# PoTaTo-Mika/fish-speech

Measured on AMD Instinct MI355X. Metric: audio-sec/wall-sec (RTF) + p50 first-sample latency, S2-Pro 4B @1/2/4/8 GPU, higher is better.
Workload: dtype bf16; 1 GPU; BASELINE config 2 per GPU: one utterance = 64-token prompt + 216 Dual-AR frames (top_k 30, top_p 0.8, temp 0.8) + codec decode [1,10,216] -> 442368 samples; global_batch=1, frames=216, prompt_len=64, first_chunk_frames=1, vocoder_chunks=first_chunk_frames, then growing 4x, vocoder=serial, parallelism=dp1

## Files before the change

fish-speech_amd/csrc/fm_kernels.h:

```cpp
#pragma once
#include <algorithm>
#include "fm_common.h"
#include "fm_tune_table.h"

enum { EPI_STORE = 0, EPI_RESID = 1, EPI_SWIGLU = 2, EPI_F32 = 3 };

template <typename T> void launch_swiglu_i8(hipStream_t s, const T* t, int ldt, T* act, int lda, int inter, int R);
template <typename T> void launch_pack(hipStream_t s, const T* src, int N, int K, T* dst);
template <typename T> void launch_quant_rows(hipStream_t s, T* w, int N, int K, int8_t* q, T* scale);
template <typename T> void launch_i8_to(hipStream_t s, const int8_t* q, int64_t n, T* dst);
void launch_pack_q8(hipStream_t s, const int8_t* src, int N, int K, int8_t* dst);
void launch_pack_q8s(hipStream_t s, const int8_t* src, int N, int K, int8_t* dst);
void launch_quant4(hipStream_t s, bf16_t* w, int N, int K, int gs, uint8_t* q, uint32_t* sz);
void launch_pack_q4(hipStream_t s, const uint8_t* q, int N, int K, uint8_t* dst);
void launch_pack_q4_rows(hipStream_t s, const uint8_t* q, int N, int K, uint32_t* dst);
void launch_pack_sz4(hipStream_t s, const uint32_t* sz, int N, int K, int gs, uint32_t* dst);
void launch_pack_q4s(hipStream_t s, const uint8_t* q, int N, int K, uint32_t* dst);

template <typename T> struct LinearArgs {
    const T* W;
    const T* W2;
    const T* bias;
    const T* X;
    int ldx, R, N, K;
// ... 212 lines not shown
    const bf16_t* nw;
    float eps;
    const bf16_t* res;
    int ldr;
    const int32_t* residx;
    int res_col, res_rows;
    bf16_t* res_out;
    bf16_t* Y;
    float* Yf;
    int N, K;
    const bf16_t* pf_kc;
    const bf16_t* pf_vc;
    const int32_t* pf_slot;
    const int32_t* pf_pos;
    size_t pf_slot_stride, pf_layer_off;
    int pf_S, pf_nkv, pf_hd;
    unsigned long long* dbg;
    int xr;
    const bf16_t* X1;
    const bf16_t* res1;
    bf16_t* res_out1;
    bf16_t* Y1;
    int skip0;
};
int rowgemv_u(int K, int qm);
void launch_rowgemv(hipStream_t s, const RowGemvArgs& a, int kind);
bool rowgemv_pair_ok(int kind, int K, bool gathered);
struct FattnWoArgs {
    FastFusedArgs<bf16_t> at;
    RowGemvArgs wo;
    uint32_t* xt;
    int gen;
    int* err;
    int delay;
    int cheap;
    int prio;
    int ilp;
    unsigned long long* dbg;
    const bf16_t* qtab;
    const int32_t* qidx;
    int qcol, qrows;
    int kv0;
    int pair;
};
bool fattn_wo_ok(int nh, int nkv, int hd, int cpos, int N, int K, int qm);
void launch_fattn_wo(hipStream_t s, const FattnWoArgs& a);
constexpr int GEMV_CHAIN_MAX = 4;
constexpr int GEMV_CHAIN_LINE = 32;
constexpr int GEMV_CHAIN_SLOTS = 17;
constexpr int GEMV_CHAIN_WORDS = GEMV_CHAIN_MAX * GEMV_CHAIN_SLOTS * GEMV_CHAIN_LINE;
enum { GEMV_CHAIN_WO_W2 = 0, GEMV_CHAIN_W13 = 1, GEMV_CHAIN_QKV = 2, GEMV_CHAIN_HEAD = 3 };
template <typename T> struct GemvChainArgs {
    GemvArgs<T> st[GEMV_CHAIN_MAX];
    int kind[GEMV_CHAIN_MAX];
    int off[GEMV_CHAIN_MAX + 1];
    int n;
    unsigned* cnt;
    int* err;
    int sleep;
};
template <typename T> void launch_gemv_chain(hipStream_t s, const GemvChainArgs<T>& c);

template <typename T> struct BstreamArgs {
    const T* W;
    const T* bias;
    const T* X;
    int ldx, R, N, K;
    T* Y;
// ... 115 lines not shown
```

fish-speech_amd/csrc/fm_llm_frame.cpp:

```cpp
#include <math.h>

#include <algorithm>
#include <array>

#include "fm_codec.h"
#include "fm_llm_model.h"

template <typename T> struct Run {
    typedef T type_t;
    fm_llm* m;
    hipStream_t s;
    int64_t E;
    bool rows_distinct_slots = false, bs_frame = false, x_ss = false;
    struct BsPending {
        bool on = false;
        const float* slab = nullptr;
        int kparts = 0, d = 0, R = 0;
        void* res = nullptr;
        void* out = nullptr;
        const void* sc = nullptr;
    } pend;
    std::vector<std::array<int, 2>> segs;
    void set_pending(const float* slab, int kparts, int d, int R, void* res, void* out, const void* sc) {
        pend = BsPending{true, slab, kparts, d, R, res, out, sc};
// ... 654 lines not shown
        int ldx_in;
        const int32_t* xidx;
        int xcol;
        void *xb, *hb;
        bool is_fast;
        int cpos, layer;
        KsbPlan kp;
        void* xo;
        int pair = 0;
        const void* x_in1 = nullptr;
    };
    static const void* row1(const Small& c, const void* p, int w) {
        return (const char*)p + (c.pair == 2 ? (size_t)w * sizeof(T) : 0);
    }
    static void* row1(const Small& c, void* p, int w) { return (char*)p + (c.pair == 2 ? (size_t)w * sizeof(T) : 0); }
    struct SmallPath {
        bool rf;
        bool fw;
        bool att_wo;
        bool row_here;
        bool tab;
        bool kv0;
        bool kv_only;
    };
    SmallPath small_path(const Small& c, bool kv_only) const {
        const StackDims& d = c.d;
        SmallPath p{};
        p.kv_only = kv_only;
        p.rf = row_fin(c.n);
        const int fq = m->quant == FM_QUANT_INT8 ? 1 : (m->quant == FM_QUANT_INT4 ? 2 : 0);
        p.fw = c.is_fast && !kv_only && p.rf && fm_tuning().fattn_wo && m->fxt && m->fdm.n_layer * m->C >= 2 &&
               m->fdm.n_layer * m->C <= 40 && fattn_wo_ok(d.nh, d.nkv, d.hd, c.cpos, d.dim, d.nq(), fq);
        p.att_wo = c.is_fast && !kv_only && fm_tuning().attn_wo && !m->quant && c.n == 1 && c.cpos < 16 && d.hd % 16 == 0 &&
                   d.hd <= 128 && d.nh % d.nkv == 0 && (d.nq() / c.kp.wo) % d.hd == 0 && d.nqkv() % 8 == 0;
        p.row_here = row_qkv(c.n) && (!c.first || (row_bits() & 16));
        const bool bits56 = sizeof(T) == 2 && !m->quant && c.is_fast && c.n == 1;
        p.tab = bits56 && c.first && c.xidx && p.fw && qkv0_live();
        p.kv0 = bits56 && c.cpos == 0 && (row_bits() & 64) && p.row_here && !p.att_wo && d.hd <= 256 &&
                (d.nqkv() - d.nq()) % fm_tuning().row_qkv_rp == 0;
        return p;
    }
    FastFusedArgs<T> small_fast_args(const Small& c, const SmallPath& p) const {
        const StackDims& d = c.d;
        FastFusedArgs<T> fa{(const T*)m->qkv, d.nqkv(), m->frame_slot, d.nh, d.nkv, d.hd, d.qk_norm,
                            m->c.norm_eps, (const T*)c.L.qn, (const T*)c.L.kn, m->frope, (T*)m->fkc,
                            (T*)m->fvc, m->fslot_stride, (size_t)c.layer * m->flayer_stride, m->C, c.cpos,
                            1.0f / sqrtf((float)d.hd), (T*)m->att};
        fa.dbg = fm_tuning().dbg;
        fa.noq = p.kv0;
        return fa;
    }
    void small_qkv(const Small& c, const SmallPath& p) {
        if (p.tab && !c.pair) return;
        const StackDims& d = c.d;
        GemvArgs<T> a = qkv_args(d, c.L, c.n);
        if (!c.is_fast && c.n == 1 && fm_tuning().kv_prefetch)
            kv_prefetch(a, (const T*)m->kc, (const T*)m->vc, m->frame_slot, m->frame_pos, m->slot_stride,
                        (size_t)c.layer * m->layer_stride, m->S, d.nkv, d.hd);
        else if (c.is_fast && c.n == 1 && fm_tuning().fkv_prefetch && m->fiota && c.cpos < 16)
            kv_prefetch(a, (const T*)m->fkc, (const T*)m->fvc, m->frame_slot, m->fiota + c.cpos, m->fslot_stride,
                        (size_t)c.layer * m->flayer_stride, m->C, d.nkv, d.hd);
        if (c.first) {
            qkv_first(d, c.L, a, c.n, c.x_in, c.ldx_in, c.pair ? nullptr : c.xidx, c.pair ? 0 : c.xcol, m->qkv,
                      p.kv0 || c.pair);
        } else if (p.row_here) {
            qkv_row(d, c.L, a, false, c.xb, 0, nullptr, 0, m->qkv, p.kv0, c.pair != 0);
        } else {
            a.X = (const T*)c.xb;
            a.ldx = d.dim;
            a.ss_in = m->ssX;
            a.ss_gran = p.rf ? 1 : 0;
            gemv(a, PRO_PRENORM, EPI_STORE, 1, "linear");
        }
    }
    void small_attn(const Small& c, const SmallPath& p) {
        const StackDims& d = c.d;
// ... 59 lines not shown
            if (!p.fw) {
                rowgemv(r, ROWGEMV_FIN);
                return;
            }
            const FastFusedArgs<T> fa = small_fast_args(c, p);
            A.at = *reinterpret_cast<const FastFusedArgs<bf16_t>*>(&fa);
            A.at.dbg = nullptr;
            A.at.row_pos = m->frame_pos;
            A.xt = m->fxt;
            A.gen = 1 + c.layer + m->fdm.n_layer * c.cpos;
            A.err = m->chain_err;
            A.delay = fm_tuning().fw_delay;
            A.cheap = fm_tuning().fw_cheap;
            A.prio = fm_tuning().fw_prio;
            A.ilp = fm_tuning().fattn_ilp;
            if (p.tab) {
                A.qtab = (const bf16_t*)m->qkv0;
                A.qidx = c.xidx;
                A.qcol = c.xcol;
                A.qrows = m->cb;
            }
            A.kv0 = p.kv0;
            A.pair = c.pair;
            hipStream_t st = s;
            auto go = [st, A] { launch_fattn_wo(st, A); };
            launch("attn", rowgemv_wbytes(r), 2.0 * r.N * r.K, go, "attn_wo");
            return;
        }
        GemvArgs<T> a = ga();
        a.W = (const T*)L.wo;
        a.bias = (const T*)L.bo;
        a.X = (const T*)m->att;
        a.ldx = d.nq();
        a.R = c.n;
        a.N = d.dim;
        a.K = d.nq();
        a.Yf = m->slabA;
        a.ldy = d.dim;
        if (c.first) {
            a.res = (const T*)c.x_in;
            a.ldr = c.ldx_in;
            a.residx = c.xidx;
            a.xidx_ld = m->C1;
            a.xidx_col = c.xcol;
            a.xidx_rows = c.xidx ? m->cb : 0;
        } else {
            a.res = (const T*)c.xb;
            a.ldr = d.dim;
        }
// ... 562 lines not shown
```

fish-speech_amd/csrc/fm_llm_model.h:

```cpp
#pragma once
#include <hip/hip_runtime.h>

#include "fm_kernels.h"
#include "fm_runtime.h"

static constexpr int PREFILL_CHUNK = 1024;
static constexpr int ATTN_PIECE = 256;
static constexpr int ATTN_SPLIT = 64;
static constexpr int GEMV_MAX_ROWS = 8;
static constexpr int KSB_MAX = 8;
static constexpr int BS_KPARTS = 8;

inline int pick_ksb(int N, int K, int R, size_t esz) {
    const int nb = (N + 15) / 16;
    const FmTuning& tu = fm_tuning();
    int ksb = 1;
    while (ksb < KSB_MAX && nb * ksb < tu.ksb_blocks && K % (32 * ksb * 2) == 0) ksb *= 2;
    if (tu.ksb_balance) {
        double best = 1e9;
        int bk = ksb;
        for (int k = 1; k <= KSB_MAX && K % (32 * k) == 0; k *= 2) {
            const int b = nb * k;
            if (b < 256) continue;
            const double rounds = (double)((b + 255) / 256), waste = rounds * 256.0 / b;
// ... 68 lines not shown
    bool use_graph = true;
    std::map<int, hipGraphExec_t> graphs;
    Profiler prof;
    std::vector<void*> allocs;
    int quant = FM_QUANT_NONE;
    int q4_gs = 0;
    int* fin_cnt = nullptr;
    float* fin_ss = nullptr;
    struct QInfo {
        const unsigned char* q8 = nullptr;
        const void* scale = nullptr;
        const uint32_t* sz = nullptr;
        const unsigned char* q8s = nullptr;
        const uint32_t* q4s = nullptr;
    };
    std::map<const void*, QInfo> qmap;
    std::map<const void*, void*> rowmajor;
    std::map<const void*, const void*> rowsz;
    std::map<const void*, const void*> rowscale;
    bool row_ok = false;
    bool row_qkv_ok = false;
    bool row_w13_ok = false;
    uint32_t* fxt = nullptr;
    void* fout_rm = nullptr;
    int32_t* fiota = nullptr;
    void* qkv0 = nullptr;
    int32_t* qkv0_iota = nullptr;
    unsigned qkv0_epoch = 0;
    bool qkv0_built = false;
    struct Prefix {
        void* buf = nullptr;
        int npos = 0;
        size_t bytes = 0;
    };
    std::map<int, Prefix> prefixes;
    int next_prefix_id = 1;
    int* pfx_slots = nullptr;
    const QInfo* qinfo(const void* W) const {
        auto it = qmap.find(W);
        return it == qmap.end() ? nullptr : &it->second;
    }

    ~fm_llm() {
        if (device >= 0) (void)hipSetDevice(device);
        for (auto& g : graphs) (void)hipGraphExecDestroy(g.second);
        for (auto& kv : w) {
// ... 37 lines not shown
```

fish-speech_amd/csrc/fm_llm_weights.cpp:

```cpp
#include "fm_llm_model.h"

void add_t(fm_llm* m, const std::string& n, int64_t rows, int64_t cols) {
    DTensor t;
    t.rows = rows;
    t.cols = cols;
    t.numel = rows * cols;
    m->w[n] = t;
}
static void add_stack(fm_llm* m, const std::string& pre, const StackDims& s) {
    for (int i = 0; i < s.n_layer; ++i) {
        std::string p = pre + std::to_string(i) + ".";
        add_t(m, p + "attention.wqkv.weight", s.nqkv(), s.dim);
        if (s.qkv_bias) add_t(m, p + "attention.wqkv.bias", 1, s.nqkv());
        add_t(m, p + "attention.wo.weight", s.dim, s.nq());
        if (s.o_bias) add_t(m, p + "attention.wo.bias", 1, s.dim);
        if (s.qk_norm) {
            add_t(m, p + "attention.q_norm.weight", 1, s.hd);
            add_t(m, p + "attention.k_norm.weight", 1, s.hd);
        }
        add_t(m, p + "feed_forward.w1.weight", s.inter, s.dim);
        add_t(m, p + "feed_forward.w3.weight", s.inter, s.dim);
        add_t(m, p + "feed_forward.w2.weight", s.dim, s.inter);
        add_t(m, p + "ffn_norm.weight", 1, s.dim);
        add_t(m, p + "attention_norm.weight", 1, s.dim);
// ... 337 lines not shown
            L.w2 = W(m, p + "feed_forward.w2.weight");
            L.an = W(m, p + "attention_norm.weight");
            L.fn = W(m, p + "ffn_norm.weight");
            auto rm = [&](const void* pk) -> void* {
                auto it = m->rowmajor.find(pk);
                return it == m->rowmajor.end() ? nullptr : it->second;
            };
            L.wo_rm = rm(L.wo);
            L.w2_rm = rm(L.w2);
            L.wqkv_rm = rm(L.wqkv);
            L.w13_rm = rm(L.w13);
        }
    };
    stack("layers.", m->sd, m->slow);
    stack("fast_layers.", m->fdm, m->fast);
    {
        int32_t io[16];
        for (int c = 0; c < 16; ++c) io[c] = c - 1;
        m->fiota = (int32_t*)m->dalloc(sizeof(io), false);
        HIPCHK(hipMemcpy(m->fiota, io, sizeof(io), hipMemcpyHostToDevice));
    }
    if (m->prec == FM_PREC_BF16)
        m->fxt = (uint32_t*)m->dalloc(2 * (size_t)m->fdm.nh * m->fdm.hd * sizeof(uint32_t));
    m->row_ok = m->row_qkv_ok = m->row_w13_ok = true;
    for (auto* st : {&m->slow, &m->fast})
        for (const LayerW& L : *st) {
            m->row_ok = m->row_ok && L.wo_rm && L.w2_rm;
            m->row_qkv_ok = m->row_qkv_ok && L.wqkv_rm;
            m->row_w13_ok = m->row_w13_ok && L.w13_rm;
        }
    if (m->quant) {
        for (auto* st : {&m->slow, &m->fast})
            for (LayerW& L : *st) L.bqkv = L.bo = nullptr;
    }
    m->emb = W(m, "embeddings.weight");
    m->cbemb = W(m, "codebook_embeddings.weight");
    m->norm = W(m, "norm.weight");
    m->fproj_w = Wopt(m, "fast_project_in.weight");
    m->fproj_b = m->quant ? nullptr : Wopt(m, "fast_project_in.bias");
    m->femb = W(m, "fast_embeddings.weight");
    m->fnorm = W(m, "fast_norm.weight");
    m->fout = W(m, "fast_output.weight");
    {
        auto it = m->rowmajor.find(m->fout);
        m->fout_rm = it == m->rowmajor.end() ? nullptr : it->second;
    }
// ... 138 lines not shown
```

fish-speech_amd/csrc/fm_rowgemv.hip:

```cpp
#include "fm_common.h"
#include "fm_kernels.h"
#include "fm_runtime.h"
#include <type_traits>

typedef __attribute__((ext_vector_type(2))) uint32_t u32x2_t;
typedef __attribute__((ext_vector_type(4))) __bf16 bf16x4_t;

__device__ __forceinline__ float dot4(u32x2_t w, u32x2_t x, float acc) {
    const bf16x4_t wb = __builtin_bit_cast(bf16x4_t, w), xb = __builtin_bit_cast(bf16x4_t, x);
    acc = __builtin_amdgcn_fdot2_f32_bf16(__builtin_shufflevector(wb, wb, 0, 1), __builtin_shufflevector(xb, xb, 0, 1),
                                          acc, false);
    acc = __builtin_amdgcn_fdot2_f32_bf16(__builtin_shufflevector(wb, wb, 2, 3), __builtin_shufflevector(xb, xb, 2, 3),
                                          acc, false);
    return acc;
}
__device__ __forceinline__ float lo16(uint32_t w) { return __uint_as_float(w << 16); }
__device__ __forceinline__ float hi16(uint32_t w) { return __uint_as_float(w & 0xffff0000u); }
__device__ __forceinline__ float dot8r(u32x4_t w, u32x4_t x, float acc) {
    const bf16x8_t wb = __builtin_bit_cast(bf16x8_t, w), xb = __builtin_bit_cast(bf16x8_t, x);
    acc = __builtin_amdgcn_fdot2_f32_bf16(__builtin_shufflevector(wb, wb, 0, 1), __builtin_shufflevector(xb, xb, 0, 1),
                                          acc, false);
    acc = __builtin_amdgcn_fdot2_f32_bf16(__builtin_shufflevector(wb, wb, 2, 3), __builtin_shufflevector(xb, xb, 2, 3),
                                          acc, false);
    acc = __builtin_amdgcn_fdot2_f32_bf16(__builtin_shufflevector(wb, wb, 4, 5), __builtin_shufflevector(xb, xb, 4, 5),
                                          acc, false);
    acc = __builtin_amdgcn_fdot2_f32_bf16(__builtin_shufflevector(wb, wb, 6, 7), __builtin_shufflevector(xb, xb, 6, 7),
                                          acc, false);
    return acc;
}
__device__ __forceinline__ void ld_pair_bf(const bf16_t* p, float& x0, float& x1) {
    const uint32_t w = *reinterpret_cast<const uint32_t*>(p);
    x0 = lo16(w);
    x1 = hi16(w);
}

template <int QM> struct RowT {
    static constexpr int EPL = QM ? 8 : 4;
    static constexpr int CE = 64 * EPL;
    using XV = typename std::conditional<QM != 0, u32x4_t, u32x2_t>::type;
    static constexpr int WPL = QM == 2 ? 1 : 2;
};

template <int U, int RP, bool PRENORM, int EPI, bool G, int QM, bool TX, int XR = 1>
__device__ __forceinline__ void rowgemv_body(const RowGemvArgs& a, const int blk, const uint32_t* xt, const uint32_t gen,
                                             int* err) {
    static_assert(!TX || (!PRENORM && EPI == 1), "tagged x: the residual form only");
    static_assert(XR == 1 || (XR == 2 && QM == 0 && EPI <= 1 && (!G || EPI == 1)), "two x rows: bf16 STORE / FIN");
    constexpr bool FIN = EPI == 1;
    using R = RowT<QM>;
    using XV = typename R::XV;
    constexpr int EPL = R::EPL, NW = EPL / 2;
    constexpr int SB = XR * 4 * RP;
    constexpr bool LATE = XR == 2 && !TX && !PRENORM && U >= 10;
    __shared__ float red[XR * (4 * RP + 8)];
    const int lane = threadIdx.x & 63, wave = threadIdx.x >> 6;
    const int n0 = blk * RP;
    const int nch = a.K / R::CE;
    const int wa = (wave * nch) >> 2, nmy = (((wave + 1) * nch) >> 2) - wa;
    const int last = nmy > 0 ? nmy - 1 : 0;
    const unsigned long long ts0 = a.dbg ? __builtin_amdgcn_s_memrealtime() : 0;
    const int er = n0 + (int)(threadIdx.x % RP);
    const int ex = XR == 2 ? (int)((threadIdx.x / RP) & 1) : 0;
    int ri = 0, xi = 0;
    if constexpr (G && FIN) {
        const int32_t iv = a.residx[a.res_col];
        ri = iv < 0 ? 0 : (iv >= a.res_rows ? a.res_rows - 1 : iv);
    } else if constexpr (G) {
        const int32_t iv = a.xidx[a.xcol];
        xi = iv < 0 ? 0 : (iv >= a.xrows ? a.xrows - 1 : iv);
    }
    bf16_t rv = 0;
    if constexpr (FIN && XR == 2) rv = ex ? a.res1[(size_t)ri * a.ldr + er] : a.res[er];
    else if constexpr (FIN) rv = a.res[(size_t)ri * a.ldr + er];
    const bf16_t bv = *(a.bias ? a.bias + er : a.X);
    bf16_t sv = 0;
    if constexpr (QM == 1) sv = a.wscale[er];
    const XV* xp = reinterpret_cast<const XV*>(a.X + (size_t)xi * a.ldx) + (size_t)wa * 64 + lane;
    const XV* gp = reinterpret_cast<const XV*>(PRENORM ? a.nw : a.X) + (size_t)wa * 64 + lane;
    XV xv[XR][U], gv[PRENORM ? U : 1];
    if constexpr (!TX) {
#pragma unroll
        for (int u = 0; u < U; ++u) {
            const int j = (u < last ? u : last) * 64;
            xv[0][u] = xp[j];
            if constexpr (XR == 2 && !LATE) xv[1][u] = (reinterpret_cast<const XV*>(a.X1) + (size_t)wa * 64 + lane)[j];
            if constexpr (PRENORM) gv[u] = gp[j];
        }
    }
    constexpr int PF = 2;
    const bool pf_on = EPI == 0 && a.pf_kc != nullptr;
    int pf_s = 0, pf_p = 0;
    if constexpr (EPI == 0) {
        pf_s = *(pf_on ? a.pf_slot : reinterpret_cast<const int32_t*>(a.X));
        pf_p = *(pf_on ? a.pf_pos : reinterpret_cast<const int32_t*>(a.X));
    }
    asm volatile("" ::: "memory");
    constexpr int WU = QM == 2 ? 1 : U, WR = QM == 2 ? 1 : RP;
    constexpr int QU = QM == 2 ? U : 1, QR = QM == 2 ? RP : 1;
    u32x2_t wv[WU][WR];
    uint32_t w4[QU][QR], szv[QU][QR];
    if constexpr (QM == 2) {
        const size_t rw = (size_t)(a.K >> 3);
        const int ng = a.K / a.gs;
        const uint32_t* wp = a.Wq4 + (size_t)n0 * rw + (size_t)wa * 64 + lane;
#pragma unroll
        for (int u = 0; u < U; ++u) {
            const int jc = u < last ? u : last;
#pragma unroll
            for (int r = 0; r < RP; ++r) {
                w4[u][r] = __builtin_nontemporal_load(wp + r * rw + jc * 64);
                szv[u][r] = a.wsz[(size_t)(n0 + r) * ng + ((wa + jc) * 512 + lane * 8) / a.gs];
            }
        }
    } else {
        const unsigned char* wb = QM ? reinterpret_cast<const unsigned char*>(a.Wq) : reinterpret_cast<const unsigned char*>(a.W);
        const size_t rowb = (size_t)a.K * (QM ? 1 : 2);
        const u32x2_t* wp = reinterpret_cast<const u32x2_t*>(wb + (size_t)n0 * rowb) + (size_t)wa * 64 + lane;
        const size_t rs8 = rowb / 8;
#pragma unroll
        for (int u = 0; u < U; ++u) {
            const int j = (u < last ? u : last) * 64;
#pragma unroll
            for (int r = 0; r < RP; ++r) wv[u][r] = __builtin_nontemporal_load(wp + r * rs8 + j);
        }
    }
    asm volatile("" ::: "memory");
    unsigned long long tsw = 0, tsx = 0;
    unsigned polls = 0;
    if constexpr (TX) {
        if (a.dbg) tsw = __builtin_amdgcn_s_memrealtime();
        const __amdgpu_buffer_rsrc_t xr = __builtin_amdgcn_make_buffer_rsrc((void*)xt, (short)0, XR * a.K * 4, 0x00020000);
        u32x4_t xw[XR][U][EPL / 4];
        for (unsigned it = 0;; ++it) {
            polls = it + 1;
#pragma unroll
            for (int x = 0; x < XR; ++x)
#pragma unroll
                for (int u = 0; u < U; ++u) {
                    const int jc = u < last ? u : last;
#pragma unroll
                    for (int q = 0; q < EPL / 4; ++q)
                        xw[x][u][q] = __builtin_amdgcn_raw_buffer_load_b128(
                            xr, (x * a.K + (wa + jc) * R::CE + EPL * lane + 4 * q) * 4, 0, 16);
                }
            bool ok = true;
#pragma unroll
// ... 3 lines not shown
#pragma unroll
                    for (int q = 0; q < EPL / 4; ++q)
#pragma unroll
                        for (int e = 0; e < 4; ++e) ok = ok && ((xw[x][u][q][e] & 0xffffu) == gen);
            if (__all(ok)) break;
            if (it >= (1u << 14)) {
                if (lane == 0) __hip_atomic_store(err, 1, __ATOMIC_RELAXED, __HIP_MEMORY_SCOPE_AGENT);
                break;
            }
            __builtin_amdgcn_s_sleep(1);
        }
        if (a.dbg) tsx = __builtin_amdgcn_s_memrealtime();
#pragma unroll
        for (int x = 0; x < XR; ++x)
#pragma unroll
            for (int u = 0; u < U; ++u)
#pragma unroll
                for (int h = 0; h < NW; ++h) {
                    const uint32_t w0 = xw[x][u][(2 * h) >> 2][(2 * h) & 3], w1 = xw[x][u][(2 * h + 1) >> 2][(2 * h + 1) & 3];
                    xv[x][u][h] = (w0 >> 16) | (w1 & 0xffff0000u);
                }
    }
    float pfw[PF];
    if constexpr (EPI == 0) {
        const char* kcb = reinterpret_cast<const char*>(pf_on ? a.pf_kc : a.X);
        const long long dv = pf_on ? reinterpret_cast<const char*>(a.pf_vc) - kcb : 0;
        const int nkv = pf_on ? a.pf_nkv : 1;
        const int b = blockIdx.x, h = b % nkv, jb = b / nkv, nb = ((int)gridDim.x - 1 - h) / nkv + 1;
        const int spr = pf_on ? a.pf_hd * 2 / 64 : 1;
        const int np = pf_on ? pf_p + 1 : 0, total = 2 * np * spr;
        const long long base = pf_on ? (long long)pf_s * (long long)a.pf_slot_stride + (long long)a.pf_layer_off +
                                           (long long)h * a.pf_S * a.pf_hd
                                     : 0;
#pragma unroll
        for (int q = 0; q < PF; ++q) {
            const int i = (jb + nb * q) * 256 + (int)threadIdx.x;
            const bool ok = i < total;
            const int ii = ok ? i : 0, row = ii / spr, sec = ii - row * spr;
            const bool isv = row >= np;
            const long long off = (isv ? dv : 0) + 2 * (base + (long long)(isv ? row - np : row) * a.pf_hd) + sec * 64;
            pfw[q] = *reinterpret_cast<const float*>(kcb + (ok ? off : 0));
        }
    }
    if constexpr (PRENORM && XR == 1) {
        float sl = 0.f;
#pragma unroll
        for (int u = 0; u < U; ++u) {
            if (u < nmy) {
#pragma unroll
                for (int h = 0; h < NW; ++h) {
                    const float e0 = lo16(xv[0][u][h]), e1 = hi16(xv[0][u][h]);
                    sl += e0 * e0 + e1 * e1;
                }
            }
        }
        sl = wave_sum(sl);
        if (lane == 0) red[4 * RP + wave] = sl;
        lds_barrier();
        const float tot = ((red[4 * RP] + red[4 * RP + 1]) + red[4 * RP + 2]) + red[4 * RP + 3];
        const float rs = 1.0f / sqrtf(tot / (float)a.K + a.eps);
#pragma unroll
        for (int u = 0; u < U; ++u) {
            XV o;
#pragma unroll
            for (int h = 0; h < NW; ++h) {
                const float y0 = bfround(bfround(lo16(xv[0][u][h]) * rs) * lo16(gv[u][h]));
                const float y1 = bfround(bfround(hi16(xv[0][u][h]) * rs) * hi16(gv[u][h]));
                o[h] = (uint32_t)f2bf(y0) | ((uint32_t)f2bf(y1) << 16);
            }
            xv[0][u] = o;
        }
    }
    if constexpr (PRENORM && XR == 2) {
#pragma unroll
        for (int x = 0; x < XR; ++x) {
            float sl = 0.f;
#pragma unroll
            for (int u = 0; u < U; ++u) {
                if (u < nmy) {
#pragma unroll
                    for (int h = 0; h < NW; ++h) {
                        const float e0 = lo16(xv[x][u][h]), e1 = hi16(xv[x][u][h]);
                        sl += e0 * e0 + e1 * e1;
// ... 64 lines not shown
#pragma unroll
                    for (int e = 0; e < 4; ++e) t = fmaf((float)((c0 >> (8 * e)) & 0xffu), xf[e], t);
#pragma unroll
                    for (int e = 0; e < 4; ++e) t = fmaf((float)((c1 >> (8 * e)) & 0xffu), xf[4 + e], t);
                    acc[0][r] = t;
                }
            }
        }
    }
    if constexpr (LATE) {
#pragma unroll
        for (int r = 0; r < RP; ++r) asm volatile("" : "+v"(acc[0][r])::"memory");
        const XV* xp1 = reinterpret_cast<const XV*>(a.X1) + (size_t)wa * 64 + lane;
#pragma unroll
        for (int u = 0; u < U; ++u) xv[1][u] = xp1[(u < last ? u : last) * 64];
#pragma unroll
        for (int u = 0; u < U; ++u) {
            if (u < nmy) {
#pragma unroll
                for (int r = 0; r < RP; ++r) acc[1][r] = dot4(wv[u][r], xv[1][u], acc[1][r]);
            }
        }
    }
    if constexpr (EPI == 0) {
#pragma unroll
        for (int q = 0; q < PF; ++q) asm volatile("" ::"v"(pfw[q]));
    }
    const unsigned long long ts1 = a.dbg ? __builtin_amdgcn_s_memrealtime() : 0;
#pragma unroll
    for (int x = 0; x < XR; ++x)
#pragma unroll
        for (int r = 0; r < RP; ++r) {
            const float v = wave_sum(acc[x][r]);
            if (lane == 0) red[(4 * x + wave) * RP + r] = v;
        }
    if constexpr (QM == 1) {
        const float v = wave_sum(xs);
        if (lane == 0) red[4 * RP + 4 + wave] = v;
    }
    __syncthreads();
    if ((int)threadIdx.x < XR * RP) {
        const int t = XR == 2 ? (int)(threadIdx.x % RP) : (int)threadIdx.x;
        const float* rd = red + 4 * RP * ex;
        float v = ((rd[t] + rd[RP + t]) + rd[2 * RP + t]) + rd[3 * RP + t];
        if constexpr (QM == 1) {
            const float xt = ((red[4 * RP + 4] + red[4 * RP + 5]) + red[4 * RP + 6]) + red[4 * RP + 7];
            v = bfround(bfround(v - 128.f * xt) * bf2f(sv));
        }
        if (a.bias) v += bf2f(bv);
        if constexpr (FIN) {
            (ex ? a.res_out1 : a.res_out)[er] = f2bf(bfround(bf2f(rv) + bfround(v)));
        } else if constexpr (EPI == 3) {
            a.Yf[er] = bfround(v);
        } else if constexpr (EPI == 2) {
            const float up = __shfl_down(v, RP / 2, 64);
            if (t < RP / 2) {
                const float g = bfround(v);
                a.Y[blockIdx.x * (RP / 2) + t] = f2bf(bfround(g / (1.0f + expf(-g))) * bfround(up));
            }
        } else if constexpr (XR == 2) {
            if (ex || er >= a.skip0) (ex ? a.Y1 : a.Y)[er] = f2bf(v);
        } else {
            a.Y[er] = f2bf(v);
        }
    }
    if (a.dbg && threadIdx.x == 0) {
#pragma unroll
        for (int x = 0; x < XR; ++x) {
            if constexpr (TX) {
                const unsigned long long t[7] = {ts0, tsw, tsx, ts1, __builtin_amdgcn_s_memrealtime(), 0, 0};
                dbg_record(a.dbg, 0xFFF8u, polls, t);
            } else {
                const unsigned long long t[7] = {ts0, ts1, __builtin_amdgcn_s_memrealtime(), 0, 0, 0, 0};
                dbg_record(a.dbg, 0xFFFAu, (unsigned)blk, t);
            }
        }
    }
}

template <int U, int RP, bool PRENORM, int EPI, bool G, int QM>
__global__ __launch_bounds__(256) __attribute__((amdgpu_waves_per_eu(RP == 2 ? 5 : 3)))
void rowgemv_kernel(RowGemvArgs a) {
    rowgemv_body<U, RP, PRENORM, EPI, G, QM, false>(a, blockIdx.x, nullptr, 0u, nullptr);
}
// ... 483 lines not shown
        fw_attend<2>(kvs, kvs + 2 * FW_MAXHD, hd, half, 1, lane, at.scale, q0, q1, k0, k1, v0, v1, o0, o1);
        const int K = at.nh * hd;
        if (in) {
            if constexpr (XR == 2) {
                const float p0 = 0.f + va0, p1 = 0.f + va1;
                const uint64_t w = (uint64_t)(((uint32_t)f2bf(p0) << 16) | gen) | ((uint64_t)(((uint32_t)f2bf(p1) << 16) | gen) << 32);
                __hip_atomic_store(reinterpret_cast<uint64_t*>(A.xt + (size_t)h * hd + 2 * lane), w, __ATOMIC_RELAXED,
                                   __HIP_MEMORY_SCOPE_AGENT);
            }
            const uint64_t w = (uint64_t)(((uint32_t)f2bf(o0) << 16) | gen) | ((uint64_t)(((uint32_t)f2bf(o1) << 16) | gen) << 32);
            __hip_atomic_store(reinterpret_cast<uint64_t*>(A.xt + K + (size_t)h * hd + 2 * lane), w, __ATOMIC_RELAXED,
                               __HIP_MEMORY_SCOPE_AGENT);
        }
        if (A.dbg && lane == 0) {
            const unsigned long long t[7] = {ts0, ts1, __builtin_amdgcn_s_memrealtime(), 0, 0, 0, 0};
#pragma unroll
            for (int x = 0; x < XR; ++x) dbg_record(A.dbg, 0xFFF9, (unsigned)h, t);
        }
        return;
    }
    rowgemv_body<U, 2, false, 1, TAB, 0, true, XR>(A.wo, (int)blockIdx.x - at.nkv, XR == 2 ? A.xt : A.xt + A.wo.K, gen, A.err);
}

bool fattn_wo_ok(int nh, int nkv, int hd, int cpos, int N, int K, int qm) {
    const int U = rowgemv_u(K, qm);
    return nkv > 0 && nh % nkv == 0 && nh / nkv <= 4 && hd % 2 == 0 && hd <= FW_MAXHD && cpos >= 0 &&
           cpos < FW_MAXJ + 1 && K == nh * hd && N % 2 == 0 && U > 0 && U <= 8;
}

void launch_fattn_wo(hipStream_t s, const FattnWoArgs& A0) {
    FattnWoArgs A = A0;
    A.dbg = fm_tuning().dbg;
    A.wo.dbg = A.dbg;
    const FastFusedArgs<bf16_t>& at = A.at;
    const int qm = A.wo.Wq4 ? 2 : (A.wo.Wq ? 1 : 0);
    FMCHECK(fattn_wo_ok(at.nh, at.nkv, at.hd, at.cpos, A.wo.N, A.wo.K, qm) && A.xt && A.err && A.gen > 0 && A.gen <= 40 && at.row_pos &&
                A.wo.res && A.wo.res_out &&
                (qm == 2 ? (A.wo.wsz && A.wo.gs % 8 == 0 && !A.wo.bias) : (qm == 1 ? (A.wo.wscale && !A.wo.bias) : A.wo.W != nullptr)),
            "fused fast attention + wo: shapes, tag and buffers");
    const dim3 grid(at.nkv + A.wo.N / 2), block(256);
    const bool G = A.wo.residx != nullptr;
    FMCHECK(!A.qtab || (qm == 0 && G && !A.kv0 && A.qidx == A.wo.residx && A.qcol == A.wo.res_col && A.qrows > 0 &&
                        A.qrows == A.wo.res_rows),
            "fused fast attention + wo: the QKV table form is bf16, gathered by the residual's index");
    FMCHECK(!A.kv0 || (qm == 0 && !G && at.cpos == 0), "fused fast attention + wo: the K / V-only form is bf16 at codebook 0");
    if (A.pair) {
        FMCHECK(qm == 0 && !A.kv0 && at.cpos == 1 && at.S >= 2 && rowgemv_pair_ok(-1, A.wo.K, false) && (A.qtab != nullptr) == G && (A.pair == 2 || (A.wo.res1 && A.wo.res_out1)),
                "fused fast attention + wo, pair form: bf16, positions 0 and 1, both rows' residuals set");
        const bool two = A.pair != 2;
        FMCHECK(two || !A.qtab, "fused fast attention + wo, pair form: the first layer is not the last");
        switch (rowgemv_u(A.wo.K, 0)) {
#define FW(u)                                                                                                            \
    case u:                                                                                                              \
        (A.qtab ? fattn_wo_pair_kernel<u, true, 2>                                                                       \
                : (two ? fattn_wo_pair_kernel<u, false, 2> : fattn_wo_pair_kernel<u, false, 1>))<<<grid, block, 0, s>>>(A); \
        break;
            FW(2) FW(3) FW(4)
            default: FW(5)
#undef FW
        }
        return;
    }
// ... 25 lines not shown
```

fish-speech_amd/csrc/fm_tune_table.h:

```cpp
#ifndef FM_TUNE_RULES
#define FM_TUNE_RULES
enum { FM_RULE_BOOL, FM_RULE_ANY, FM_RULE_SET, FM_RULE_RANGE, FM_RULE_MULT16 };
template <typename... V> constexpr int fm_knob_set(V... v) { return (0 | ... | (1 << v)); }
#define FM_BOOL FM_RULE_BOOL, 0, 0
#define FM_ANY FM_RULE_ANY, 0, 0
#define FM_SET(...) FM_RULE_SET, fm_knob_set(__VA_ARGS__), 0
#define FM_RANGE(lo, hi) FM_RULE_RANGE, lo, hi
#define FM_MIN(lo) FM_RULE_RANGE, lo, 0x7fffffff
#define FM_MULT16 FM_RULE_MULT16, 0, 0
#define FM_ZERO_OR_MULT16 FM_RULE_MULT16, 1, 0
#endif

#ifdef FM_KNOB
FM_KNOB(gemv_nt, 1, FM_BOOL)
FM_KNOB(gemv_u, 8, FM_SET(2, 4, 8))
FM_KNOB(gemv_wpb, 4, FM_SET(4, 8))
FM_KNOB(sampler_kth, 1, FM_BOOL)
FM_KNOB(sampler_fast, 1, FM_BOOL)
FM_KNOB(attn_cap, 32, FM_ZERO_OR_MULT16)
FM_KNOB(attn_wo, 0, FM_BOOL)
FM_KNOB(ksb_blocks, 512, FM_MIN(1))
FM_KNOB(batched_fused_attn, 1, FM_BOOL)
FM_KNOB(attn_cap_batched, 128, FM_ZERO_OR_MULT16)
FM_KNOB(linear_u32, 4, FM_SET(4, 8))
// ... 41 lines not shown
FM_KNOB(chain_max, 4, FM_RANGE(2, 4))
FM_KNOB(chain_sleep, 4, FM_SET(1, 4, 16))
FM_KNOB(gemv_chain, 0, FM_BOOL)
FM_KNOB(bs_xfirst, 1, FM_BOOL)
FM_KNOB(bs_vec_epi, 1, FM_BOOL)
FM_KNOB(bsacc_kparts, 0, FM_SET(0, 1, 2, 4, 8))
FM_KNOB(q_u, 4, FM_SET(2, 4, 8, 16))
FM_KNOB(fin8, 1, FM_BOOL)
FM_KNOB(fin_split, 0, FM_RANGE(0, 16))
FM_KNOB(bstream_q8, 1, FM_BOOL)
FM_KNOB(bstream_q4, 1, FM_BOOL)
FM_KNOB(int4_stream, 1, FM_BOOL)
FM_KNOB(fw_delay, 0, FM_RANGE(0, 1000))
FM_KNOB(fw_cheap, 0, FM_BOOL)
FM_KNOB(fw_prio, 0, FM_BOOL)
FM_KNOB(fattn_wo, 1, FM_BOOL)
FM_KNOB(fattn_ilp, 1, FM_BOOL)
FM_KNOB(row_qkv_rp, 8, FM_SET(4, 8, 16))
FM_KNOB(rowgemv_q4, 31, FM_RANGE(0, 31))
FM_KNOB(rowgemv, 123, FM_RANGE(0, 127))
FM_KNOB(row_copies, 1, FM_BOOL)
FM_KNOB(prefix_vec, 1, FM_BOOL)
FM_KNOB(fast_pair, 1, FM_BOOL)
#endif
```

Measured before the change: 12.16 audio-sec/wall-sec.

## Fuse fast-transformer QKV row GEMV into the fused attention+wo kernel

New measurement: 12.20 audio-sec/wall-sec, median of 6. About the same (+0.4%).

```diff
diff --git a/fish-speech_amd/csrc/fm_kernels.h b/fish-speech_amd/csrc/fm_kernels.h
--- a/fish-speech_amd/csrc/fm_kernels.h
+++ b/fish-speech_amd/csrc/fm_kernels.h
@@ -258,6 +258,7 @@
     bf16_t* res_out1;
     bf16_t* Y1;
     int skip0;
+    uint32_t* yt;
 };
 int rowgemv_u(int K, int qm);
 void launch_rowgemv(hipStream_t s, const RowGemvArgs& a, int kind);
@@ -278,8 +279,12 @@
     int qcol, qrows;
     int kv0;
     int pair;
+    int fqkv;
+    RowGemvArgs qkv;
+    uint32_t* qt;
 };
 bool fattn_wo_ok(int nh, int nkv, int hd, int cpos, int N, int K, int qm);
+bool fqkv_ok(int nh, int nkv, int hd, int cpos, int N, int K, int dim, int nqkv);
 void launch_fattn_wo(hipStream_t s, const FattnWoArgs& a);
 constexpr int GEMV_CHAIN_MAX = 4;
 constexpr int GEMV_CHAIN_LINE = 32;
diff --git a/fish-speech_amd/csrc/fm_llm_frame.cpp b/fish-speech_amd/csrc/fm_llm_frame.cpp
--- a/fish-speech_amd/csrc/fm_llm_frame.cpp
+++ b/fish-speech_amd/csrc/fm_llm_frame.cpp
@@ -700,6 +700,7 @@
         bool tab;
         bool kv0;
         bool kv_only;
+        bool fq;
     };
     SmallPath small_path(const Small& c, bool kv_only) const {
         const StackDims& d = c.d;
@@ -716,6 +717,8 @@
         p.tab = bits56 && c.first && c.xidx && p.fw && qkv0_live();
         p.kv0 = bits56 && c.cpos == 0 && (row_bits() & 64) && p.row_here && !p.att_wo && d.hd <= 256 &&
                 (d.nqkv() - d.nq()) % fm_tuning().row_qkv_rp == 0;
+        p.fq = bits56 && p.fw && !c.first && c.cpos >= 2 && p.row_here && !c.pair && !p.kv0 && !p.kv_only && !p.tab && !p.att_wo &&
+               fm_tuning().fqkv_fuse && m->fqt && fqkv_ok(d.nh, d.nkv, d.hd, c.cpos, d.dim, d.nq(), d.dim, d.nqkv());
         return p;
     }
     FastFusedArgs<T> small_fast_args(const Small& c, const SmallPath& p) const {
@@ -730,6 +733,7 @@
     }
     void small_qkv(const Small& c, const SmallPath& p) {
         if (p.tab && !c.pair) return;
+        if (p.fq) return;
         const StackDims& d = c.d;
         GemvArgs<T> a = qkv_args(d, c.L, c.n);
         if (!c.is_fast && c.n == 1 && fm_tuning().kv_prefetch)
@@ -835,9 +839,26 @@
             }
             A.kv0 = p.kv0;
             A.pair = c.pair;
+            int64_t bytes = rowgemv_wbytes(r);
+            double flops = 2.0 * r.N * r.K;
+            if (p.fq) {
+                RowGemvArgs& q = A.qkv;
+                row_weight(q, L.wqkv_rm, L.wqkv);
+                q.X = (const bf16_t*)c.xb;
+                q.bias = (const bf16_t*)L.bqkv;
+                q.nw = (const bf16_t*)L.an;
+                q.eps = m->c.norm_eps;
+                q.Y = (bf16_t*)m->qkv;
+                q.N = d.nqkv();
+                q.K = d.dim;
+                A.fqkv = 1;
+                A.qt = m->fqt;
+                bytes += rowgemv_wbytes(q) + (int64_t)q.K * 2;
+                flops += 2.0 * q.N * q.K;
+            }
             hipStream_t st = s;
             auto go = [st, A] { launch_fattn_wo(st, A); };
-            launch("attn", rowgemv_wbytes(r), 2.0 * r.N * r.K, go, "attn_wo");
+            launch("attn", bytes, flops, go, "attn_wo");
             return;
         }
         GemvArgs<T> a = ga();
diff --git a/fish-speech_amd/csrc/fm_llm_model.h b/fish-speech_amd/csrc/fm_llm_model.h
--- a/fish-speech_amd/csrc/fm_llm_model.h
+++ b/fish-speech_amd/csrc/fm_llm_model.h
@@ -114,6 +114,7 @@
     bool row_qkv_ok = false;
     bool row_w13_ok = false;
     uint32_t* fxt = nullptr;
+    uint32_t* fqt = nullptr;
     void* fout_rm = nullptr;
     int32_t* fiota = nullptr;
     void* qkv0 = nullptr;
diff --git a/fish-speech_amd/csrc/fm_llm_weights.cpp b/fish-speech_amd/csrc/fm_llm_weights.cpp
--- a/fish-speech_amd/csrc/fm_llm_weights.cpp
+++ b/fish-speech_amd/csrc/fm_llm_weights.cpp
@@ -383,6 +383,7 @@
     }
     if (m->prec == FM_PREC_BF16)
         m->fxt = (uint32_t*)m->dalloc(2 * (size_t)m->fdm.nh * m->fdm.hd * sizeof(uint32_t));
+    if (m->prec == FM_PREC_BF16) m->fqt = (uint32_t*)m->dalloc((size_t)m->fdm.nqkv() * sizeof(uint32_t));
     m->row_ok = m->row_qkv_ok = m->row_w13_ok = true;
     for (auto* st : {&m->slow, &m->fast})
         for (const LayerW& L : *st) {
diff --git a/fish-speech_amd/csrc/fm_rowgemv.hip b/fish-speech_amd/csrc/fm_rowgemv.hip
--- a/fish-speech_amd/csrc/fm_rowgemv.hip
+++ b/fish-speech_amd/csrc/fm_rowgemv.hip
@@ -41,11 +41,13 @@
     static constexpr int WPL = QM == 2 ? 1 : 2;
 };
 
-template <int U, int RP, bool PRENORM, int EPI, bool G, int QM, bool TX, int XR = 1>
+template <int U, int RP, bool PRENORM, int EPI, bool G, int QM, bool TX, int XR = 1, bool TY = false>
 __device__ __forceinline__ void rowgemv_body(const RowGemvArgs& a, const int blk, const uint32_t* xt, const uint32_t gen,
                                              int* err) {
     static_assert(!TX || (!PRENORM && EPI == 1), "tagged x: the residual form only");
     static_assert(XR == 1 || (XR == 2 && QM == 0 && EPI <= 1 && (!G || EPI == 1)), "two x rows: bf16 STORE / FIN");
+    static_assert(!TY || (EPI == 0 && XR == 1 && QM == 0 && !TX), "tagged y: the one-row bf16 STORE form only");
+    constexpr bool PFK = EPI == 0 && !TY;
     constexpr bool FIN = EPI == 1;
     using R = RowT<QM>;
     using XV = typename R::XV;
@@ -53,6 +55,7 @@
     constexpr int SB = XR * 4 * RP;
     constexpr bool LATE = XR == 2 && !TX && !PRENORM && U >= 10;
     __shared__ float red[XR * (4 * RP + 8)];
+    __shared__ bf16_t bsh[TY ? RP : 1];
     const int lane = threadIdx.x & 63, wave = threadIdx.x >> 6;
     const int n0 = blk * RP;
     const int nch = a.K / R::CE;
@@ -88,9 +91,9 @@
         }
     }
     constexpr int PF = 2;
-    const bool pf_on = EPI == 0 && a.pf_kc != nullptr;
+    const bool pf_on = PFK && a.pf_kc != nullptr;
     int pf_s = 0, pf_p = 0;
-    if constexpr (EPI == 0) {
+    if constexpr (PFK) {
         pf_s = *(pf_on ? a.pf_slot : reinterpret_cast<const int32_t*>(a.X));
         pf_p = *(pf_on ? a.pf_pos : reinterpret_cast<const int32_t*>(a.X));
     }
@@ -117,11 +120,22 @@
         const size_t rowb = (size_t)a.K * (QM ? 1 : 2);
         const u32x2_t* wp = reinterpret_cast<const u32x2_t*>(wb + (size_t)n0 * rowb) + (size_t)wa * 64 + lane;
         const size_t rs8 = rowb / 8;
+        if constexpr (TY) {
+            const __amdgpu_buffer_rsrc_t wr = __builtin_amdgcn_make_buffer_rsrc(
+                (void*)(wb + (size_t)n0 * rowb), (short)0, (int)(RP * rowb), 0x00020000);
+#pragma unroll
+            for (int u = 0; u < U; ++u) {
+                const int vo = ((wa + (u < last ? u : last)) * 64 + lane) * 8;
+#pragma unroll
+                for (int r = 0; r < RP; ++r) wv[u][r] = __builtin_amdgcn_raw_buffer_load_b64(wr, vo, r * (int)rowb, 2);
+            }
+        } else {
 #pragma unroll
         for (int u = 0; u < U; ++u) {
             const int j = (u < last ? u : last) * 64;
 #pragma unroll
             for (int r = 0; r < RP; ++r) wv[u][r] = __builtin_nontemporal_load(wp + r * rs8 + j);
+        }
         }
     }
     asm volatile("" ::: "memory");
@@ -171,7 +185,7 @@
                 }
     }
     float pfw[PF];
-    if constexpr (EPI == 0) {
+    if constexpr (PFK) {
         const char* kcb = reinterpret_cast<const char*>(pf_on ? a.pf_kc : a.X);
         const long long dv = pf_on ? reinterpret_cast<const char*>(a.pf_vc) - kcb : 0;
         const int nkv = pf_on ? a.pf_nkv : 1;
@@ -205,9 +219,18 @@
         }
         sl = wave_sum(sl);
         if (lane == 0) red[4 * RP + wave] = sl;
+        if constexpr (TY) {
+            if ((int)threadIdx.x < RP) bsh[threadIdx.x] = bv;
+        }
         lds_barrier();
         const float tot = ((red[4 * RP] + red[4 * RP + 1]) + red[4 * RP + 2]) + red[4 * RP + 3];
         const float rs = 1.0f / sqrtf(tot / (float)a.K + a.eps);
+        if constexpr (TY) {
+#pragma unroll
+            for (int u = 0; u < U; ++u)
+#pragma unroll
+                for (int h = 0; h < NW; ++h) asm volatile("" : "+v"(xv[0][u][h]));
+        }
 #pragma unroll
         for (int u = 0; u < U; ++u) {
             XV o;
@@ -318,7 +341,7 @@
             }
         }
     }
-    if constexpr (EPI == 0) {
+    if constexpr (PFK) {
 #pragma unroll
         for (int q = 0; q < PF; ++q) asm volatile("" ::"v"(pfw[q]));
     }
@@ -343,7 +366,7 @@
             const float xt = ((red[4 * RP + 4] + red[4 * RP + 5]) + red[4 * RP + 6]) + red[4 * RP + 7];
             v = bfround(bfround(v - 128.f * xt) * bf2f(sv));
         }
-        if (a.bias) v += bf2f(bv);
+        if (a.bias) v += bf2f(TY ? bsh[TY ? t : 0] : bv);
         if constexpr (FIN) {
             (ex ? a.res_out1 : a.res_out)[er] = f2bf(bfround(bf2f(rv) + bfround(v)));
         } else if constexpr (EPI == 3) {
@@ -356,6 +379,10 @@
             }
         } else if constexpr (XR == 2) {
             if (ex || er >= a.skip0) (ex ? a.Y1 : a.Y)[er] = f2bf(v);
+        } else if constexpr (TY) {
+            const bf16_t y = f2bf(v);
+            __hip_atomic_store(a.yt + er, ((uint32_t)y << 16) | gen, __ATOMIC_RELAXED, __HIP_MEMORY_SCOPE_AGENT);
+            a.Y[er] = y;
         } else {
             a.Y[er] = f2bf(v);
         }
@@ -885,6 +912,179 @@
     rowgemv_body<U, 2, false, 1, TAB, 0, true, XR>(A.wo, (int)blockIdx.x - at.nkv, XR == 2 ? A.xt : A.xt + A.wo.K, gen, A.err);
 }
 
+template <int UQ, int U>
+__global__ __launch_bounds__(256) __attribute__((amdgpu_waves_per_eu(6)))
+void fqkv_attn_wo_kernel(FattnWoArgs A) {
+    __shared__ __attribute__((aligned(16))) bf16_t kvs[2 * FW_MAXJ * FW_MAXHD];
+    const FastFusedArgs<bf16_t>& at = A.at;
+    const uint32_t gen = ((uint32_t)A.at.row_pos[0] * 41u + (uint32_t)A.gen) % 65535u + 1u;
+    if ((int)blockIdx.x < at.nkv) {
+        const unsigned long long ts0 = A.dbg ? __builtin_amdgcn_s_memrealtime() : 0;
+        const int lane = threadIdx.x & 63, wave = threadIdx.x >> 6;
+        if (A.prio) __builtin_amdgcn_s_setprio(3);
+        const int kvh = blockIdx.x, hd = at.hd, g = at.nh / at.nkv, cpos = at.cpos, half = hd >> 1;
+        const int slot = at.row_slot[0];
+        const bool live = wave < g, in = lane < half;
+        const int h = kvh * g + (live ? wave : 0), pp = in ? lane : 0;
+        const float* tab = at.rope + (size_t)cpos * hd;
+        const size_t base = (size_t)slot * at.slot_stride + at.layer_off + (size_t)kvh * at.S * hd;
+        const int nck = cpos * hd / 8;
+        auto kv_src = [&](int i) {
+            const bool ok = i < 2 * nck, isv = ok && i >= nck;
+            const int c = ok ? (isv ? i - nck : i) : 0;
+            return reinterpret_cast<const u32x4_t*>((isv ? at.vc : at.kc) + base + (size_t)c * 8);
+        };
+        auto kv_dst = [&](int i) {
+            const bool isv = i >= nck;
+            return reinterpret_cast<u32x4_t*>(kvs + (isv ? FW_MAXJ * FW_MAXHD : 0) + (isv ? i - nck : i) * 8);
+        };
+        u32x4_t kvr[2];
+#pragma unroll
+        for (int q = 0; q < 2; ++q) kvr[q] = *kv_src((int)threadIdx.x + 256 * q);
+        float qw0, qw1, kw0, kw1;
+        ld_pair_bf(at.qk_norm ? at.qn + 2 * pp : reinterpret_cast<const bf16_t*>(tab), qw0, qw1);
+        ld_pair_bf(at.qk_norm ? at.kn + 2 * pp : reinterpret_cast<const bf16_t*>(tab), kw0, kw1);
+        const float c_ = tab[2 * pp], s_ = tab[2 * pp + 1];
+        asm volatile("" ::: "memory");
+        const __amdgpu_buffer_rsrc_t qr = __builtin_amdgcn_make_buffer_rsrc((void*)A.qt, (short)0, at.ldqkv * 4, 0x00020000);
+        const int oq = (h * hd + 2 * pp) * 4, ok_ = ((at.nh + kvh) * hd + 2 * pp) * 4,
+                  ov = ((at.nh + at.nkv + kvh) * hd + 2 * pp) * 4;
+        u32x2_t wq, wk, wv;
+        unsigned polls = 0;
+        for (unsigned it = 0;; ++it) {
+            polls = it + 1;
+            wq = __builtin_amdgcn_raw_buffer_load_b64(qr, oq, 0, 16);
+            wk = __builtin_amdgcn_raw_buffer_load_b64(qr, ok_, 0, 16);
+            wv = __builtin_amdgcn_raw_buffer_load_b64(qr, ov, 0, 16);
+            const bool cur = (wq[0] & 0xffffu) == gen && (wq[1] & 0xffffu) == gen && (wk[0] & 0xffffu) == gen &&
+                             (wk[1] & 0xffffu) == gen && (wv[0] & 0xffffu) == gen && (wv[1] & 0xffffu) == gen;
+            if (__all(cur)) break;
+            if (it >= (1u << 14)) {
+                if (lane == 0) __hip_atomic_store(A.err, 1, __ATOMIC_RELAXED, __HIP_MEMORY_SCOPE_AGENT);
+                break;
+            }
+            __builtin_amdgcn_s_sleep(1);
+        }
+        const unsigned long long tsq = A.dbg ? __builtin_amdgcn_s_memrealtime() : 0;
+        float q0 = in ? hi16(wq[0]) : 0.f, q1 = in ? hi16(wq[1]) : 0.f;
+        float k0 = in ? hi16(wk[0]) : 0.f, k1 = in ? hi16(wk[1]) : 0.f;
+        const float v0 = in ? hi16(wv[0]) : 0.f, v1 = in ? hi16(wv[1]) : 0.f;
+#pragma unroll
+        for (int q = 0; q < 2; ++q)
+            if ((int)threadIdx.x + 256 * q < 2 * nck) *kv_dst((int)threadIdx.x + 256 * q) = kvr[q];
+        if (at.qk_norm) {
+            float sq = 0.f, sk = 0.f;
+            sq += q0 * q0 + q1 * q1;
+            sk += k0 * k0 + k1 * k1;
+            sq = wave_sum(sq);
+            sk = wave_sum(sk);
+            const float rq = 1.0f / sqrtf(sq / (float)hd + at.eps), rk = 1.0f / sqrtf(sk / (float)hd + at.eps);
+            q0 = bfround((q0 * rq) * qw0);
+            q1 = bfround((q1 * rq) * qw1);
+            k0 = bfround((k0 * rk) * kw0);
+            k1 = bfround((k1 * rk) * kw1);
+        }
+        {
+            const float a0 = bfround(q0 * c_ - q1 * s_), a1 = bfround(q1 * c_ + q0 * s_);
+            const float b0 = bfround(k0 * c_ - k1 * s_), b1 = bfround(k1 * c_ + k0 * s_);
+            q0 = a0;
+            q1 = a1;
+            k0 = b0;
+            k1 = b1;
+        }
+        if (wave == 0 && in) {
+            bf16_t* kd = at.kc + base + (size_t)cpos * hd;
+            bf16_t* vd = at.vc + base + (size_t)cpos * hd;
+            *reinterpret_cast<uint32_t*>(kd + 2 * lane) = (uint32_t)f2bf(k0) | ((uint32_t)f2bf(k1) << 16);
+            *reinterpret_cast<uint32_t*>(vd + 2 * lane) = (uint32_t)f2bf(v0) | ((uint32_t)f2bf(v1) << 16);
+        }
+        __syncthreads();
+        const unsigned long long ts1 = A.dbg ? __builtin_amdgcn_s_memrealtime() : 0;
+        if (!live) return;
+        const bf16_t* Ks = kvs;
+        const bf16_t* Vs = kvs + FW_MAXJ * FW_MAXHD;
+        float o0 = 0.f, o1 = 0.f;
+#define FWA(n) fw_attend<n>(Ks, Vs, hd, half, cpos, lane, at.scale, q0, q1, k0, k1, v0, v1, o0, o1)
+        switch (cpos) {
+            case 0: FWA(1); break;
+            case 1: FWA(2); break;
+            case 2: FWA(3); break;
+            case 3: FWA(4); break;
+            case 4: FWA(5); break;
+            case 5: FWA(6); break;
+            case 6: FWA(7); break;
+            case 7: FWA(8); break;
+            case 8: FWA(9); break;
+            case 9: FWA(10); break;
+            case 10: case 11: FWA(12); break;
+            default: FWA(16); break;
+        }
+#undef FWA
+        if (in) {
+            const uint64_t w = (uint64_t)(((uint32_t)f2bf(o0) << 16) | gen) | ((uint64_t)(((uint32_t)f2bf(o1) << 16) | gen) << 32);
+            __hip_atomic_store(reinterpret_cast<uint64_t*>(A.xt + (size_t)h * hd + 2 * lane), w, __ATOMIC_RELAXED,
+                               __HIP_MEMORY_SCOPE_AGENT);
+        }
+        if (A.dbg && lane == 0) {
+            const unsigned long long te = __builtin_amdgcn_s_memrealtime();
+            const unsigned long long t[7] = {ts0, ts1, te, 0, 0, 0, 0};
+            dbg_record(A.dbg, 0xFFF9, (unsigned)h, t);
+            const unsigned long long tq[7] = {ts0, tsq, ts1, te, 0, 0, 0};
+            dbg_record(A.dbg, 0xFFF7, polls, tq);
+        }
+        return;
+    }
+    const int blk = (int)blockIdx.x - at.nkv, nqb = A.qkv.N / 8;
+    if (blk < nqb) {
+        rowgemv_body<UQ, 8, true, 0, false, 0, false, 1, true>(A.qkv, blk, nullptr, gen, nullptr);
+    } else {
+        const __amdgpu_buffer_rsrc_t qr = __builtin_amdgcn_make_buffer_rsrc((void*)A.qt, (short)0, A.qkv.N * 4, 0x00020000);
+        const int off = ((blk - nqb) % nqb) * 32;
+        for (unsigned it = 0; it < (1u << 14); ++it) {
+            const uint32_t w = __builtin_amdgcn_raw_buffer_load_b32(qr, off, 0, 16);
+            if ((w & 0xffffu) == gen) break;
+            __builtin_amdgcn_s_sleep(4);
+        }
+    }
+    rowgemv_body<U, 2, false, 1, false, 0, true>(A.wo, blk, A.xt, gen, A.err);
+}
+
+static int fqkv_num_cus() {
+    static int n = 0;
+    if (!n) {
+        int dev = 0;
+        (void)hipGetDevice(&dev);
+        if (hipDeviceGetAttribute(&n, hipDeviceAttributeMultiprocessorCount, dev) != hipSuccess || n <= 0) n = 1;
+    }
+    return n;
+}
+
+bool fqkv_ok(int nh, int nkv, int hd, int cpos, int N, int K, int dim, int nqkv) {
+    const int UQ = rowgemv_u(dim, 0), U = rowgemv_u(K, 0);
+    return fattn_wo_ok(nh, nkv, hd, cpos, N, K, 0) && (UQ == 2 || UQ == 3) && U >= 2 && U <= 4 && nqkv == (nh + 2 * nkv) * hd &&
+           nqkv % 8 == 0 && nqkv / 8 <= N / 2 && nkv + N / 2 <= 6 * fqkv_num_cus();
+}
+
+static void launch_fqkv_attn_wo(hipStream_t s, FattnWoArgs& A) {
+    const FastFusedArgs<bf16_t>& at = A.at;
+    FMCHECK(fqkv_ok(at.nh, at.nkv, at.hd, at.cpos, A.wo.N, A.wo.K, A.qkv.K, A.qkv.N) && A.wo.W && !A.wo.residx && !A.qtab &&
+                !A.kv0 && !A.pair && A.wo.xr != 2 && A.qt && A.qkv.W && !A.qkv.Wq && !A.qkv.Wq4 && !A.qkv.xidx && A.qkv.X &&
+                A.qkv.nw && A.qkv.Y && at.ldqkv == A.qkv.N,
+            "fused QKV + fast attention + wo: bf16, one row, not the first layer, shapes and buffers");
+    A.qkv.dbg = A.dbg;
+    A.qkv.yt = A.qt;
+    if (!A.qkv.ldx) A.qkv.ldx = A.qkv.K;
+    const dim3 grid(at.nkv + A.wo.N / 2), block(256);
+    const int UQ = rowgemv_u(A.qkv.K, 0);
+    switch (rowgemv_u(A.wo.K, 0)) {
+#define FQ(u) \
+    case u: (UQ == 2 ? fqkv_attn_wo_kernel<2, u> : fqkv_attn_wo_kernel<3, u>)<<<grid, block, 0, s>>>(A); break;
+        FQ(2) FQ(3)
+        default: FQ(4)
+#undef FQ
+    }
+}
+
 bool fattn_wo_ok(int nh, int nkv, int hd, int cpos, int N, int K, int qm) {
     const int U = rowgemv_u(K, qm);
     return nkv > 0 && nh % nkv == 0 && nh / nkv <= 4 && hd % 2 == 0 && hd <= FW_MAXHD && cpos >= 0 &&
@@ -901,6 +1101,10 @@
                 A.wo.res && A.wo.res_out &&
                 (qm == 2 ? (A.wo.wsz && A.wo.gs % 8 == 0 && !A.wo.bias) : (qm == 1 ? (A.wo.wscale && !A.wo.bias) : A.wo.W != nullptr)),
             "fused fast attention + wo: shapes, tag and buffers");
+    if (A.fqkv) {
+        launch_fqkv_attn_wo(s, A);
+        return;
+    }
     const dim3 grid(at.nkv + A.wo.N / 2), block(256);
     const bool G = A.wo.residx != nullptr;
     FMCHECK(!A.qtab || (qm == 0 && G && !A.kv0 && A.qidx == A.wo.residx && A.qcol == A.wo.res_col && A.qrows > 0 &&
diff --git a/fish-speech_amd/csrc/fm_tune_table.h b/fish-speech_amd/csrc/fm_tune_table.h
--- a/fish-speech_amd/csrc/fm_tune_table.h
+++ b/fish-speech_amd/csrc/fm_tune_table.h
@@ -87,4 +87,5 @@
 FM_KNOB(row_copies, 1, FM_BOOL)
 FM_KNOB(prefix_vec, 1, FM_BOOL)
 FM_KNOB(fast_pair, 1, FM_BOOL)
+FM_KNOB(fqkv_fuse, 1, FM_BOOL)
 #endif
```
